# GitHubOfAndrew/TeAMOFlow

Hardware: AMD Instinct MI355X
Metric: train_interactions_per_sec (higher is better)
Workload: dtype f32

## Files before the change

teamoflow_amd/csrc/tmf_wmrb.hip:

```cpp
#include <math.h>
#include <stdlib.h>

#include <type_traits>

#include "tmf_common.h"

namespace tmf {

constexpr int kThreads = 256;
constexpr int kWaves = kThreads / 64;
constexpr int kPosChunk = 512;
constexpr int kUnrollW = 4;
constexpr int kG4Unroll = 4;

__host__ __device__ inline int round4(int x) { return (x + 3) & ~3; }

__host__ __device__ inline int sp_padded(int S) {
    const int nf4 = (S + 3) / 4;
    const int per = ((nf4 + 2 * kWaves - 1) / (2 * kWaves) + 1) & ~1;
    return 4 * 2 * kWaves * per;
}

__device__ __forceinline__ void count_ge0_x4(int& c0, int& c1, float x0, float x1, float x2, float x3) {
    unsigned long long m0, m1, m2, m3;
// ... 995 lines not shown
__global__ __launch_bounds__(64 * (kS5Waves + 1)) void k_wmrb_scores5(const int32_t* __restrict__ ids, const int32_t* __restrict__ outs,
                                                                     const int64_t* __restrict__ wg_ptr, int64_t wg0, int64_t n_users,
                                                                     const T* __restrict__ U, const T* __restrict__ V,
                                                                     float* __restrict__ sp, float* __restrict__ p, S5Pace pace) {
    constexpr int G = 32, NGB = 2 * kS5Waves;
    constexpr uint32_t RB = RowBytes<G, NV, T>::value;
    extern __shared__ __attribute__((aligned(16))) char smem_raw[];
    __shared__ int s_win[kS5Waves];
    __shared__ int s_gate;
    int* wst = reinterpret_cast<int*>(smem_raw + (size_t)kS5Users * RB);
    const int tid = threadIdx.x, lane = tid & 63, wave = tid >> 6, g = lane & (G - 1), gid = tid / G;
    const int64_t wg = wg0 + blockIdx.x;
    const int64_t ubeg = wg * kS5Users;
    const int nu = (int)((n_users - ubeg < kS5Users) ? n_users - ubeg : kS5Users);
    const bool paced = pace.cnt != nullptr;
    {
        const tmf_f4* src = reinterpret_cast<const tmf_f4*>(reinterpret_cast<const char*>(U) + ubeg * (int64_t)RB);
        tmf_f4* dst = reinterpret_cast<tmf_f4*>(smem_raw);
        for (int i = tid; i < nu * (int)(RB / 16); i += 64 * (kS5Waves + 1)) dst[i] = __builtin_nontemporal_load(src + i);
        if (paced)
            for (int i = tid; i <= pace.nw; i += 64 * (kS5Waves + 1)) wst[i] = pace.wst[wg * (pace.nw + 1) + i];
        if (tid < kS5Waves) s_win[tid] = 0;
        if (tid == 0) s_gate = paced ? pace.lag : INT32_MAX;
    }
    __syncthreads();
    if (wave == kS5Waves) {
        if (!paced) return;
        const int x = blockIdx.x & 7, peers = ((int)gridDim.x - x + 7) / 8;
        int* cnt = pace.cnt + (size_t)x * pace.nw * kS5Stride;
        int published = 0, gate = pace.lag, idle = 0;
        bool open = false;
        for (;;) {
            int mn = (lane < kS5Waves) ? __hip_atomic_load(&s_win[lane], __ATOMIC_RELAXED, __HIP_MEMORY_SCOPE_WORKGROUP) : INT32_MAX;
#pragma unroll
            for (int o = 8; o >= 1; o >>= 1) mn = min(mn, __shfl_xor(mn, o, 64));
            mn = __builtin_amdgcn_readfirstlane(mn);
            const bool done = mn == INT32_MAX;
            const int target = done ? pace.nw : mn;
            if (lane == 0)
                for (int w = published; w < target; ++w) __hip_atomic_fetch_add(cnt + (size_t)w * kS5Stride, 1, __ATOMIC_RELAXED, __HIP_MEMORY_SCOPE_AGENT);
            if (target > published) published = target;
            if (done) return;
            if (!open && gate < pace.nw - 1) {
                int c = (lane == 0) ? __hip_atomic_load(cnt + (size_t)(gate - pace.lag) * kS5Stride, __ATOMIC_RELAXED, __HIP_MEMORY_SCOPE_AGENT) : 0;
                c = __builtin_amdgcn_readfirstlane(c);
                if (c >= peers) {
                    ++gate;
                    idle = 0;
                    if (lane == 0) __hip_atomic_store(&s_gate, gate, __ATOMIC_RELAXED, __HIP_MEMORY_SCOPE_WORKGROUP);
                    continue;
                }
                if (++idle > 4000) {
                    open = true;
                    if (lane == 0) __hip_atomic_store(&s_gate, INT32_MAX, __ATOMIC_RELAXED, __HIP_MEMORY_SCOPE_WORKGROUP);
                }
            }
            __builtin_amdgcn_s_sleep(4);
        }
    }
    const int64_t beg = wg_ptr[wg], end = wg_ptr[wg + 1];
    const int steps = (int)((end - beg) >> 3);
    const uint32_t loff = 16u * (uint32_t)g;
    const int my_entry = Reduce8x32::entry_of_lane(lane);
    const bool owner = Reduce8x32::owner(lane);
    const int4* id4 = reinterpret_cast<const int4*>(ids + beg);
    const int32_t* out8 = outs + beg + my_entry;
    const int mine = steps > gid ? (steps - gid + NGB - 1) / NGB : 0;
    const int rounds = __builtin_amdgcn_readfirstlane(mine);
    if (rounds > 0) {
        const int last = mine > 0 ? gid + NGB * (mine - 1) : 0;
        struct Ids {
            int4 a, b;
            int o;
        };
        auto fetch = [&](int i) {
            const int st = gid + NGB * i;
            const int sc = st <= last ? st : last;
            Ids r{id4[2 * sc], id4[2 * sc + 1], out8[8 * sc]};
            if (i >= mine) r.o = kS5Pad;
            return r;
        };
        int cur_w = 0, next_b = paced ? wst[1] : INT32_MAX;
        auto pace_to = [&](int i) {
            if (!paced || i >= rounds || cur_w >= pace.nw - 1) return;
            const int st_w = __builtin_amdgcn_readfirstlane(gid + NGB * i);
            if (st_w < next_b) return;
            do {
                ++cur_w;
                next_b = wst[cur_w + 1];
            } while (st_w >= next_b && cur_w < pace.nw - 1);
            if (lane == 0) __hip_atomic_store(&s_win[wave], cur_w, __ATOMIC_RELAXED, __HIP_MEMORY_SCOPE_WORKGROUP);
            for (int spin = 0; spin < 20000; ++spin) {
                if (__hip_atomic_load(&s_gate, __ATOMIC_RELAXED, __HIP_MEMORY_SCOPE_WORKGROUP) >= cur_w) break;
                __builtin_amdgcn_s_sleep(2);
            }
        };
        auto gather = [&](Raw<NV, T> (&y)[8], const Ids& d) {
            const int idv[8] = {d.a.x, d.a.y, d.a.z, d.a.w, d.b.x, d.b.y, d.b.z, d.b.w};
#pragma unroll
            for (int t = 0; t < 8; ++t) load_raw32<G, NV>(y[t], V, (uint32_t)idv[t] & 0xffffffu, loff);
        };
        auto finish = [&](const Raw<NV, T> (&y)[8], const Ids& d) {
            const int idv[8] = {d.a.x, d.a.y, d.a.z, d.a.w, d.b.x, d.b.y, d.b.z, d.b.w};
            float pr[8];
#pragma unroll
            for (int t = 0; t < 8; ++t) {
                Raw<NV, T> x;
                const char* xr = smem_raw + ((uint32_t)idv[t] >> 24) * RB + loff;
                if constexpr (std::is_same<T, float>::value) {
#pragma unroll
                    for (int v = 0; v < NV; ++v) x.v[v] = *reinterpret_cast<const float4*>(xr + 16 * G * v);
                } else {
#pragma unroll
                    for (int pv = 0; pv < NV / 2; ++pv) x.v[pv] = *reinterpret_cast<const bf16x8*>(xr + 16 * G * pv);
                }
                pr[t] = dot_raw<NV>(x, y[t]);
            }
            const float sc = Reduce8x32::run(pr, lane);
            if (owner && d.o != kS5Pad) __builtin_nontemporal_store(sc, d.o >= 0 ? sp + d.o : p + ~d.o);
        };
        Raw<NV, T> yA[8], yB[8];
        Ids A = fetch(0);
        Ids B = fetch(1);
        pace_to(0);
        gather(yA, A);
        for (int i = 0; i < rounds; i += 2) {
            Ids C = fetch(i + 2);
            __builtin_amdgcn_sched_barrier(0);
            pace_to(i + 1);
            gather(yB, B);
            __builtin_amdgcn_sched_barrier(0);
            finish(yA, A);
            __builtin_amdgcn_sched_barrier(0);
            if (i + 1 >= rounds) break;
            Ids Dn = fetch(i + 3);
            __builtin_amdgcn_sched_barrier(0);
            pace_to(i + 2);
            gather(yA, C);
            __builtin_amdgcn_sched_barrier(0);
            finish(yB, B);
            __builtin_amdgcn_sched_barrier(0);
            A = C;
            B = Dn;
        }
    }
    if (lane == 0) __hip_atomic_store(&s_win[wave], INT32_MAX, __ATOMIC_RELAXED, __HIP_MEMORY_SCOPE_WORKGROUP);
}

}

namespace tmf {
constexpr int kS6Users = 64;
constexpr int kS6Waves = 8;

template <int NV, typename T>
__global__ __launch_bounds__(64 * kS6Waves) void k_wmrb_scores6(const int32_t* __restrict__ ids, const int32_t* __restrict__ outs,
                                                                const int64_t* __restrict__ chunk_ptr, int64_t chunk0, int64_t n_groups,
                                                                int64_t n_users, const T* __restrict__ U, const T* __restrict__ V,
                                                                float* __restrict__ sp, float* __restrict__ p) {
    constexpr int G = 32, NGB = 2 * kS6Waves;
    constexpr uint32_t RB = RowBytes<G, NV, T>::value;
    __shared__ __attribute__((aligned(16))) char smem_raw[kS6Users * RB];
    const int tid = threadIdx.x, lane = tid & 63, g = lane & (G - 1), gid = tid / G;
    const int64_t chunk = chunk0 + blockIdx.x;
    const int64_t beg = chunk_ptr[chunk], end = chunk_ptr[chunk + 1];
    if (beg == end) return;
    const int64_t ubeg = (chunk % n_groups) * kS6Users;
    const int nu = (int)((n_users - ubeg < kS6Users) ? n_users - ubeg : kS6Users);
    {
        const tmf_f4* src = reinterpret_cast<const tmf_f4*>(reinterpret_cast<const char*>(U) + ubeg * (int64_t)RB);
        tmf_f4* dst = reinterpret_cast<tmf_f4*>(smem_raw);
        for (int i = tid; i < nu * (int)(RB / 16); i += 64 * kS6Waves) dst[i] = __builtin_nontemporal_load(src + i);
    }
    __syncthreads();
    const int steps = (int)((end - beg) >> 3);
    const uint32_t loff = 16u * (uint32_t)g;
    const int my_entry = Reduce8x32::entry_of_lane(lane);
    const bool owner = Reduce8x32::owner(lane);
    const int4* id4 = reinterpret_cast<const int4*>(ids + beg);
    const int32_t* out8 = outs + beg + my_entry;
    const int mine = steps > gid ? (steps - gid + NGB - 1) / NGB : 0;
    const int rounds = __builtin_amdgcn_readfirstlane(mine);
    if (rounds == 0) return;
    const int last = mine > 0 ? gid + NGB * (mine - 1) : 0;
    struct Ids {
        int4 a, b;
        int o;
    };
    auto fetch = [&](int i) {
        const int st = gid + NGB * i;
        const int sc = st <= last ? st : last;
        Ids r{id4[2 * sc], id4[2 * sc + 1], out8[8 * sc]};
        if (i >= mine) r.o = kS5Pad;
        return r;
    };
    auto gather = [&](Raw<NV, T> (&y)[8], const Ids& d) {
        const int idv[8] = {d.a.x, d.a.y, d.a.z, d.a.w, d.b.x, d.b.y, d.b.z, d.b.w};
#pragma unroll
        for (int t = 0; t < 8; ++t) load_raw32<G, NV>(y[t], V, (uint32_t)idv[t] & 0xffffffu, loff);
    };
    auto finish = [&](const Raw<NV, T> (&y)[8], const Ids& d) {
        const int idv[8] = {d.a.x, d.a.y, d.a.z, d.a.w, d.b.x, d.b.y, d.b.z, d.b.w};
        float pr[8];
#pragma unroll
        for (int t = 0; t < 8; ++t) {
            Raw<NV, T> x;
            const char* xr = smem_raw + ((uint32_t)idv[t] >> 24) * RB + loff;
            if constexpr (std::is_same<T, float>::value) {
#pragma unroll
                for (int v = 0; v < NV; ++v) x.v[v] = *reinterpret_cast<const float4*>(xr + 16 * G * v);
            } else {
#pragma unroll
                for (int pv = 0; pv < NV / 2; ++pv) x.v[pv] = *reinterpret_cast<const bf16x8*>(xr + 16 * G * pv);
            }
            pr[t] = dot_raw<NV>(x, y[t]);
        }
        const float sc = Reduce8x32::run(pr, lane);
        if (owner && d.o != kS5Pad) __builtin_nontemporal_store(sc, d.o >= 0 ? sp + d.o : p + ~d.o);
    };
    Raw<NV, T> yA[8];
    Ids A = fetch(0);
    for (int i = 0; i < rounds; ++i) {
        Ids B = fetch(i + 1);
        __builtin_amdgcn_sched_barrier(0);
        gather(yA, A);
        __builtin_amdgcn_sched_barrier(0);
        finish(yA, A);
        A = B;
    }
}

}

static bool s6_supported(int n_components, int bf16, int64_t n_items) {
    const tmf::RowGeom geom = bf16 ? tmf::row_geom_bf16(n_components) : tmf::row_geom(n_components);
    const int64_t row_bytes = (int64_t)geom.ld * (bf16 ? 2 : 4);
    return geom.G == 32 && n_items > 0 && n_items < (1 << 24) && n_items * row_bytes < ((int64_t)1 << 32);
}

template <typename T>
static int wmrb_scores6_impl(const int32_t* ids, const int32_t* outs, const int64_t* chunk_ptr, int64_t n_groups, int32_t n_slices,
                             int64_t n_users, int64_t n_items, const void* U, const void* V, float* sp, float* p, int n_components,
                             void* stream) {
    if (n_users == 0 || n_slices == 0) return TMF_OK;
    const RowGeom geom = row_geom_of<T>(n_components);
    TMF_REQUIRE(ids && outs && chunk_ptr && U && V && sp && p, "wmrb_scores6: null pointer");
    TMF_REQUIRE(n_groups == (n_users + kS6Users - 1) / kS6Users && n_slices > 0, "wmrb_scores6: %lld groups for %lld users (%d per group), %d slices",
                (long long)n_groups, (long long)n_users, kS6Users, n_slices);
    if (!s6_supported(n_components, std::is_same<T, __bf16>::value, n_items)) {
        set_error("wmrb_scores6: needs rows of 32 lanes (fp32 65..128 / bf16 129..256 components) and fewer than 2^24 items in a table "
                  "below 4 GB (got %d components, %lld items)", n_components, (long long)n_items);
        return TMF_E_UNSUPPORTED;
    }
    const int64_t per_slice = n_groups * 64 * kS6Waves;
    const int max_slices = (int)((((int64_t)1 << 32) - 1) / per_slice);
    TMF_REQUIRE(max_slices >= 1, "wmrb_scores6: %lld user groups exceed one launch", (long long)n_groups);
    for (int s0 = 0; s0 < n_slices; s0 += max_slices) {
        const int nsl = (n_slices - s0 < max_slices) ? n_slices - s0 : max_slices;
        const unsigned blocks = (unsigned)(n_groups * nsl);
#define CALL(G_, NV_)                                                                                                       \
    {                                                                                                                       \
        if constexpr (G_ == 32) {                                                                                           \
            hipLaunchKernelGGL((k_wmrb_scores6<NV_, T>), dim3(blocks), dim3(64 * kS6Waves), 0, (hipStream_t)stream, ids, outs, \
                               chunk_ptr, (int64_t)s0 * n_groups, n_groups, n_users, (const T*)U, (const T*)V, sp, p);      \
        }                                                                                                                   \
    }
        TMF_DISPATCH(T, geom, CALL);
#undef CALL
    }
    return check_launch("tmf_wmrb_scores6");
}

namespace tmf {
constexpr int kS7Users = 256;
constexpr int kS7Slots = 6144;
constexpr int kS7K = 4;
constexpr int kS7Waves = 16;
constexpr int kS7Flight = 2;
constexpr uint32_t kS7RowBytes = 512;
constexpr size_t kS7Lds = (size_t)kS7Users * kS7RowBytes + (size_t)(kS7Slots + 64) * sizeof(float);

struct S7Streams {
    const int4* steps;
    const int32_t* place;
    const int64_t* sub_step;
    const int64_t* sub_place;
    const int32_t* chunk_sub;
    const int32_t* sub_wave;
    const int32_t* sub_fill;
};

__global__ __launch_bounds__(64 * kS7Waves) void k_wmrb_scores7(S7Streams a, int64_t chunk0, int64_t n_groups, int64_t n_users,
                                                                const float* __restrict__ U, const float* __restrict__ V,
                                                                float* __restrict__ sp, float* __restrict__ p) {
    constexpr int NG = 8 * kS7Waves, NT = 64 * kS7Waves, FL = kS7Flight;
    extern __shared__ __attribute__((aligned(16))) char smem_raw[];
    float* sbuf = reinterpret_cast<float*>(smem_raw + (size_t)kS7Users * kS7RowBytes);
    const int tid = threadIdx.x, lane = tid & 63, g = lane & 7, gid = tid >> 3;
    const int64_t chunk = chunk0 + blockIdx.x;
    const int sub_b = a.chunk_sub[chunk], sub_e = a.chunk_sub[chunk + 1];
    if (sub_b == sub_e) return;
    const int64_t ubeg = (chunk % n_groups) * kS7Users;
    const int nu = (int)((n_users - ubeg < kS7Users) ? n_users - ubeg : kS7Users);
    {
        const tmf_f4* src = reinterpret_cast<const tmf_f4*>(reinterpret_cast<const char*>(U) + ubeg * (int64_t)kS7RowBytes);
        tmf_f4* dst = reinterpret_cast<tmf_f4*>(smem_raw);
        for (int i = tid; i < nu * (int)(kS7RowBytes / 16); i += NT) dst[i] = __builtin_nontemporal_load(src + i);
    }
    __syncthreads();
    const uint32_t par = (lane >> 4) & 1;
    const uint32_t offA = 16u * g + 128u * par, offB = 16u * g + 128u * (par ^ 1u);
    const uint32_t slot_sel = 0x0c0c0000u | ((2u * (g & 3) + 1u) << 8) | (2u * (g & 3));
    struct Row {
        float4 v[4];
    };
    auto dot = [](const Row& x, const Row& y) {
        float q[4];
#pragma unroll
        for (int v = 0; v < 4; ++v) {
            tmf_f2 a = tmf_f2{x.v[v].x, x.v[v].y} * tmf_f2{y.v[v].x, y.v[v].y};
            a = __builtin_elementwise_fma(tmf_f2{x.v[v].z, x.v[v].w}, tmf_f2{y.v[v].z, y.v[v].w}, a);
            q[v] = a.x + a.y;
        }
        return (q[0] + q[2]) + (q[1] + q[3]);
    };
    auto run = [&](auto fill_tag, const int4* rec0, int first, int stride, int end, int rounds) {
        constexpr int FILL = decltype(fill_tag)::value;
        auto fetch = [&](int i) {
            const int st = first + stride * i;
            return rec0[st < end ? st : end - 1];
        };
        auto gather = [&](Row& y, const int4& r) {
            const char* base = reinterpret_cast<const char*>(V);
            const uint32_t oa = row_byte_off<kS7RowBytes>((uint32_t)r.x, offA), ob = row_byte_off<kS7RowBytes>((uint32_t)r.x, offB);
            y.v[0] = *reinterpret_cast<const float4*>(base + oa);
            y.v[1] = *reinterpret_cast<const float4*>(base + ob);
            y.v[2] = *reinterpret_cast<const float4*>(base + oa + 256);
            y.v[3] = *reinterpret_cast<const float4*>(base + ob + 256);
        };
        auto finish = [&](const Row& y, const int4& r, int i) {
            float s[FILL];
#pragma unroll
            for (int k = 0; k < FILL; ++k) {
                const uint32_t lu = ((uint32_t)r.y >> (8 * k)) & 0xffu;
                const char* xa = smem_raw + (lu * kS7RowBytes + offA);
                const char* xb = smem_raw + (lu * kS7RowBytes + offB);
                Row x;
                x.v[0] = *reinterpret_cast<const float4*>(xa);
                x.v[1] = *reinterpret_cast<const float4*>(xb);
                x.v[2] = *reinterpret_cast<const float4*>(xa + 256);
                x.v[3] = *reinterpret_cast<const float4*>(xb + 256);
                float t = dot(x, y);
                t += TMF_DPP_MOV(t, 0xB1);
                t += TMF_DPP_MOV(t, 0x4E);
                t += TMF_DPP_MOV(t, 0x141);
                s[k] = t;
            }
            float mine_s = s[0];
            if constexpr (FILL == 2) mine_s = (g & 1) ? s[1] : s[0];
            if constexpr (FILL == 3) mine_s = (g & 2) ? s[2] : ((g & 1) ? s[1] : s[0]);
            if constexpr (FILL == 4) mine_s = (g & 2) ? ((g & 1) ? s[3] : s[2]) : ((g & 1) ? s[1] : s[0]);
            uint32_t slot = __builtin_amdgcn_perm((uint32_t)r.w, (uint32_t)r.z, slot_sel);
            slot = (slot < (uint32_t)kS7Slots && first + stride * i < end) ? slot : (uint32_t)kS7Slots;
            if (g < FILL) sbuf[slot] = mine_s;
        };
        Row y[FL];
        int4 rec[2 * FL];
#pragma unroll
        for (int j = 0; j < FL; ++j) rec[j] = fetch(j);
#pragma unroll
        for (int j = 0; j < FL; ++j) {
            gather(y[j], rec[j]);
            rec[FL + j] = fetch(FL + j);
        }
        int i = 0;
        for (; i + 2 * FL <= rounds; i += 2 * FL) {
#pragma unroll
            for (int j = 0; j < 2 * FL; ++j) {
                __builtin_amdgcn_sched_barrier(0);
                finish(y[j % FL], rec[j], i + j);
                __builtin_amdgcn_sched_barrier(0);
                gather(y[j % FL], rec[(j + FL) % (2 * FL)]);
                rec[j] = fetch(i + j + 2 * FL);
            }
        }
        const int rem = rounds - i;
#pragma unroll
        for (int j = 0; j < 2 * FL - 1; ++j) {
            if (j < rem) {
                __builtin_amdgcn_sched_barrier(0);
                finish(y[j % FL], rec[j], i + j);
                __builtin_amdgcn_sched_barrier(0);
                if (j + FL < rem) gather(y[j % FL], rec[j + FL]);
            }
        }
    };
    const int wave = __builtin_amdgcn_readfirstlane(tid >> 6);
    const bool by_fill = a.sub_wave != nullptr;
    for (int sub = sub_b; sub < sub_e; ++sub) {
        const int64_t st0 = a.sub_step[sub];
        const int nsteps = (int)(a.sub_step[sub + 1] - st0);
        const int64_t pl0 = a.sub_place[sub];
        const int nslots = (int)(a.sub_place[sub + 1] - pl0);
        const int4* rec0 = a.steps + st0;
        const int32_t* pl = a.place + pl0;
        int32_t where[kS7Slots / NT];
#pragma unroll
        for (int q = 0; q < kS7Slots / NT; ++q) where[q] = (tid + NT * q < nslots) ? __builtin_nontemporal_load(pl + tid + NT * q) : 0;
        int lo = 8 * wave, hi = nsteps, stride = NG, wb = 0, we = 0, cls = 0;
        if (by_fill) {
            const int32_t* sw = a.sub_wave + (int64_t)sub * (kS7Waves + 1) + wave;
            wb = __builtin_amdgcn_readfirstlane(sw[0]);
            we = __builtin_amdgcn_readfirstlane(sw[1]);
            cls = __builtin_amdgcn_readfirstlane(a.sub_fill[(int64_t)sub * kS7K]);
            lo = wb, hi = we < cls ? we : cls, stride = 8;
        }
        if (lo < hi) run(std::integral_constant<int, 4>{}, rec0, lo + (by_fill ? (gid & 7) : gid - 8 * wave), stride, hi, (hi - lo + stride - 1) / stride);
        if (by_fill) {
            const int32_t* sf = a.sub_fill + (int64_t)sub * kS7K;
            int end = cls + __builtin_amdgcn_readfirstlane(sf[1]);
            lo = wb > cls ? wb : cls, hi = we < end ? we : end, cls = end;
            if (lo < hi) run(std::integral_constant<int, 3>{}, rec0, lo + (gid & 7), 8, hi, (hi - lo + 7) / 8);
            end = cls + __builtin_amdgcn_readfirstlane(sf[2]);
            lo = wb > cls ? wb : cls, hi = we < end ? we : end, cls = end;
            if (lo < hi) run(std::integral_constant<int, 2>{}, rec0, lo + (gid & 7), 8, hi, (hi - lo + 7) / 8);
            lo = wb > cls ? wb : cls, hi = we;
            if (lo < hi) run(std::integral_constant<int, 1>{}, rec0, lo + (gid & 7), 8, hi, (hi - lo + 7) / 8);
        }
        __syncthreads();
#pragma unroll
        for (int q = 0; q < kS7Slots / NT; ++q)
            if (tid + NT * q < nslots)
                __builtin_nontemporal_store(sbuf[tid + NT * q], where[q] >= 0 ? sp + where[q] : p + ~where[q]);
        __syncthreads();
    }
}

}

static bool s7_supported(int n_components, int bf16, int64_t n_items) {
    return !bf16 && n_components >= 65 && n_components <= 128 && s6_supported(n_components, 0, n_items);
}

static int wmrb_scores7_impl(const void* steps, const int32_t* place, const int64_t* sub_step, const int64_t* sub_place,
                             const int32_t* chunk_sub, const int32_t* sub_wave, const int32_t* sub_fill, int64_t n_groups, int32_t n_slices, int64_t n_users, int64_t n_items,
                             const void* U, const void* V, float* sp, float* p, int n_components, void* stream) {
    if (n_users == 0 || n_slices == 0) return TMF_OK;
    TMF_REQUIRE(steps && place && sub_step && sub_place && chunk_sub && U && V && sp && p, "wmrb_scores7: null pointer");
    TMF_REQUIRE(!sub_wave == !sub_fill, "wmrb_scores7: sub_wave and sub_fill come together");
    TMF_REQUIRE(n_groups == (n_users + kS7Users - 1) / kS7Users && n_slices > 0, "wmrb_scores7: %lld groups for %lld users (%d per group), %d slices",
                (long long)n_groups, (long long)n_users, kS7Users, n_slices);
    if (!s7_supported(n_components, 0, n_items)) {
        set_error("wmrb_scores7: needs fp32 rows of 65..128 components and fewer than 2^24 items in a table below 4 GB "
                  "(got %d components, %lld items)", n_components, (long long)n_items);
        return TMF_E_UNSUPPORTED;
    }
    static LdsGrant grant;
    if (int rc = grant_dynamic_lds(reinterpret_cast<const void*>(&k_wmrb_scores7), kS7Lds, grant)) return rc;
    const S7Streams a{static_cast<const int4*>(steps), place, sub_step, sub_place, chunk_sub, sub_wave, sub_fill};
    const int64_t per_slice = n_groups * 64 * kS7Waves;
    const int max_slices = (int)((((int64_t)1 << 32) - 1) / per_slice);
    TMF_REQUIRE(max_slices >= 1, "wmrb_scores7: %lld user groups exceed one launch", (long long)n_groups);
    for (int s0 = 0; s0 < n_slices; s0 += max_slices) {
        const int nsl = (n_slices - s0 < max_slices) ? n_slices - s0 : max_slices;
        hipLaunchKernelGGL(k_wmrb_scores7, dim3((unsigned)(n_groups * nsl)), dim3(64 * kS7Waves), kS7Lds, (hipStream_t)stream, a,
                           (int64_t)s0 * n_groups, n_groups, n_users, (const float*)U, (const float*)V, sp, p);
    }
    return check_launch("tmf_wmrb_scores7");
}

static int s5_launches(int64_t n_wg, int wgs_per_launch) { return (int)((n_wg + wgs_per_launch - 1) / wgs_per_launch); }
static int s5_wgs_per_launch(int wgs_per_launch) {
    if (wgs_per_launch > 0) return wgs_per_launch;
    int dev = 0, cus = 256;
    if (hipGetDevice(&dev) == hipSuccess) (void)hipDeviceGetAttribute(&cus, hipDeviceAttributeMultiprocessorCount, dev);
    return cus > 0 ? cus : 256;
}

template <typename T>
static int wmrb_scores5_impl(const int32_t* ids, const int32_t* outs, const int64_t* wg_ptr, int64_t n_wg, int64_t n_users,
                             int64_t n_items, const void* U, const void* V, float* sp, float* p, int n_components,
                             int wgs_per_launch, const int32_t* wstart, int32_t n_windows, int lag, void* workspace,
                             size_t workspace_bytes, void* stream) {
    if (n_wg == 0 || n_users == 0) return TMF_OK;
    const RowGeom geom = row_geom_of<T>(n_components);
    TMF_REQUIRE(ids && outs && wg_ptr && U && V && sp && p, "wmrb_scores5: null pointer");
    TMF_REQUIRE(n_wg == (n_users + kS5Users - 1) / kS5Users, "wmrb_scores5: %lld workgroups for %lld users (%d per workgroup)",
                (long long)n_wg, (long long)n_users, kS5Users);
    const size_t row_bytes = (size_t)geom.ld * sizeof(T);
    if (geom.G != 32 || row_bytes * kS5Users > 128 * 1024 || n_items <= 0 || n_items >= (1 << 24) ||
        (int64_t)n_items * (int64_t)row_bytes >= ((int64_t)1 << 32)) {
        set_error("wmrb_scores5: needs rows of 32 lanes (fp32 65..128 / bf16 129..256 components) and fewer than 2^24 items "
                  "in a table below 4 GB (got %d components, %lld items)", n_components, (long long)n_items);
        return TMF_E_UNSUPPORTED;
    }
    wgs_per_launch = s5_wgs_per_launch(wgs_per_launch);
    const int launches = s5_launches(n_wg, wgs_per_launch);
    const bool paced = wstart != nullptr && workspace != nullptr && n_windows > 1;
    const size_t per_launch = (size_t)8 * (paced ? n_windows : 0) * kS5Stride * sizeof(int);
    if (paced) {
        TMF_REQUIRE(n_windows <= kS5MaxWindows && lag >= 0, "wmrb_scores5: %d windows (at most %d), lag %d", n_windows, kS5MaxWindows, lag);
        TMF_REQUIRE(workspace_bytes >= per_launch * launches, "wmrb_scores5: workspace of %zu bytes needed, got %zu", per_launch * launches,
                    workspace_bytes);
        if (hipMemsetAsync(workspace, 0, per_launch * launches, (hipStream_t)stream) != hipSuccess) {
            set_error("wmrb_scores5: hipMemsetAsync failed");
            return TMF_E_LAUNCH;
        }
    }
    const size_t lds = row_bytes * kS5Users + (paced ? (size_t)(n_windows + 1) * sizeof(int) : 0);
#define CALL(G_, NV_)                                                                                                       \
    {                                                                                                                       \
        if constexpr (G_ == 32) {                                                                                           \
            static LdsGrant grant;                                                                                          \
            if (int rc = grant_dynamic_lds(reinterpret_cast<const void*>(&k_wmrb_scores5<NV_, T>), lds, grant)) return rc;  \
            for (int l = 0; l < launches; ++l) {                                                                            \
                const int64_t w0 = (int64_t)l * wgs_per_launch;                                                             \
                const unsigned blocks = (unsigned)((n_wg - w0 < wgs_per_launch) ? n_wg - w0 : wgs_per_launch);              \
                const S5Pace pace{wstart, paced ? reinterpret_cast<int*>(static_cast<char*>(workspace) + per_launch * l) : nullptr, \
                                  n_windows, lag};                                                                          \
                hipLaunchKernelGGL((k_wmrb_scores5<NV_, T>), dim3(blocks), dim3(64 * (kS5Waves + 1)), lds, (hipStream_t)stream, \
                                   ids, outs, wg_ptr, w0, n_users, (const T*)U, (const T*)V, sp, p, pace);                  \
            }                                                                                                               \
        }                                                                                                                   \
    }
    TMF_DISPATCH(T, geom, CALL);
#undef CALL
    return check_launch("tmf_wmrb_scores5");
}

template <typename T>
static int wmrb_finish_impl(const float* part, int32_t n_slices, int32_t n_users, const void* U_old, void* U_out,
                            int n_components, int epi, tmf_adam adam, void* stream) {
    if (n_users == 0) return TMF_OK;
    TMF_REQUIRE(part && U_out && n_slices > 0 && (epi == TMF_EPI_GRAD || U_old), "wmrb_finish: bad arguments");
    TMF_REQUIRE(epi == TMF_EPI_ADAM || epi == TMF_EPI_GRAD, "wmrb_finish: bad epilogue %d", epi);
    const RowGeom geom = row_geom_of<T>(n_components);
#define CALL(G_, NV_)                                                                                                  \
    {                                                                                                                  \
        constexpr int per_block = (64 / G_) * kWaves;                                                                  \
        hipLaunchKernelGGL((k_wmrb_finish<G_, NV_, T>), dim3((unsigned)(((int64_t)n_users + per_block - 1) / per_block)), \
                           dim3(kThreads), 0, (hipStream_t)stream, part, (int)n_slices, (int64_t)n_users,                \
                           (const T*)U_old, U_out, epi, adam);                                                         \
    }
    TMF_DISPATCH(T, geom, CALL);
#undef CALL
    return check_launch("tmf_wmrb_finish");
}

#define TMF_SLICED_ENTRY_POINTS(SFX, T_)                                                                                  \
    extern "C" int tmf_wmrb_scores3_##SFX(const tmf_slice_lists* lists, const void* U, const void* V, float* sp, float* p, \
                                          int n_components, void* stream) {                                               \
        return wmrb_scores3_impl<T_>(lists, U, V, sp, p, n_components, stream);                                           \
    }                                                                                                                     \
    extern "C" int tmf_wmrb_scores5_##SFX(const int32_t* ids, const int32_t* outs, const int64_t* wg_ptr, int64_t n_wg,    \
                                          int64_t n_users, int64_t n_items, const void* U, const void* V, float* sp,      \
                                          float* p, int n_components, int wgs_per_launch, const int32_t* wstart,          \
                                          int32_t n_windows, int lag, void* workspace, size_t workspace_bytes,            \
                                          void* stream) {                                                                 \
        return wmrb_scores5_impl<T_>(ids, outs, wg_ptr, n_wg, n_users, n_items, U, V, sp, p, n_components, wgs_per_launch, \
                                     wstart, n_windows, lag, workspace, workspace_bytes, stream);                         \
    }                                                                                                                     \
    extern "C" int tmf_wmrb_scores6_##SFX(const int32_t* ids, const int32_t* outs, const int64_t* chunk_ptr, int64_t n_groups, \
                                          int32_t n_slices, int64_t n_users, int64_t n_items, const void* U, const void* V, \
                                          float* sp, float* p, int n_components, void* stream) {                          \
        return wmrb_scores6_impl<T_>(ids, outs, chunk_ptr, n_groups, n_slices, n_users, n_items, U, V, sp, p, n_components, stream); \
    }                                                                                                                     \
    extern "C" int tmf_wmrb_gradu3_##SFX(const tmf_slice_lists* lists, const float* D, const float* delta,                \
                                         const void* V, float* part, int per_slice_launches, int n_components,            \
                                         void* stream) {                                                                  \
        return wmrb_gradu3_impl<T_>(lists, D, delta, V, part, per_slice_launches, n_components, stream);                  \
    }                                                                                                                     \
    extern "C" int tmf_wmrb_gradu4_##SFX(const tmf_slice_lists* lists, const float* D, const float* delta, const void* V,  \
                                         const void* U_old, void* U_out, int n_components, int epi, tmf_adam adam,       \
                                         int32_t users_per_launch, void* workspace, size_t workspace_bytes, void* stream) { \
        return wmrb_gradu4_impl<T_>(lists, D, delta, V, U_old, U_out, n_components, epi, adam, users_per_launch, workspace, \
                                    workspace_bytes, stream);                                                            \
    }                                                                                                                     \
    extern "C" int tmf_wmrb_finish_##SFX(const float* part, int32_t n_slices, int32_t n_users, const void* U_old,         \
                                         void* U_out, int n_components, int epi, tmf_adam adam, void* stream) {           \
        return wmrb_finish_impl<T_>(part, n_slices, n_users, U_old, U_out, n_components, epi, adam, stream);               \
    }

TMF_SLICED_ENTRY_POINTS(f32, float)
TMF_SLICED_ENTRY_POINTS(bf16, __bf16)

extern "C" int tmf_wmrb_scores6_users_per_group(void) { return tmf::kS6Users; }
extern "C" int tmf_wmrb_scores6_supported(int n_components, int bf16, int64_t n_items) { return s6_supported(n_components, bf16, n_items); }
extern "C" int tmf_wmrb_scores7_f32(const void* steps, const int32_t* place, const int64_t* sub_step, const int64_t* sub_place,
                                    const int32_t* chunk_sub, int64_t n_groups, int32_t n_slices, int64_t n_users, int64_t n_items,
                                    const void* U, const void* V, float* sp, float* p, int n_components, void* stream) {
    return wmrb_scores7_impl(steps, place, sub_step, sub_place, chunk_sub, nullptr, nullptr, n_groups, n_slices, n_users, n_items, U, V, sp, p,
                             n_components, stream);
}
extern "C" int tmf_wmrb_scores7_fill_f32(const void* steps, const int32_t* place, const int64_t* sub_step, const int64_t* sub_place,
                                         const int32_t* chunk_sub, const int32_t* sub_wave, const int32_t* sub_fill, int64_t n_groups,
                                         int32_t n_slices, int64_t n_users, int64_t n_items, const void* U, const void* V, float* sp,
                                         float* p, int n_components, void* stream) {
    TMF_REQUIRE(sub_wave && sub_fill, "wmrb_scores7_fill: null pointer");
    return wmrb_scores7_impl(steps, place, sub_step, sub_place, chunk_sub, sub_wave, sub_fill, n_groups, n_slices, n_users, n_items, U, V,
                             sp, p, n_components, stream);
}
extern "C" int tmf_wmrb_scores7_waves(void) { return tmf::kS7Waves; }
extern "C" int tmf_wmrb_scores7_users_per_group(void) { return tmf::kS7Users; }
extern "C" int tmf_wmrb_scores7_slots(void) { return tmf::kS7Slots; }
extern "C" int tmf_wmrb_scores7_supported(int n_components, int bf16, int64_t n_items) { return s7_supported(n_components, bf16, n_items); }
extern "C" int tmf_wmrb_scores5_users_per_workgroup(void) { return tmf::kS5Users; }
extern "C" size_t tmf_wmrb_scores5_workspace_bytes(int64_t n_wg, int32_t n_windows, int wgs_per_launch) {
    if (n_wg <= 0 || n_windows <= 1) return 0;
    return (size_t)s5_launches(n_wg, s5_wgs_per_launch(wgs_per_launch)) * 8 * (size_t)n_windows * tmf::kS5Stride * sizeof(int);
}
extern "C" int tmf_wmrb_scores5_supported(int n_components, int bf16, int64_t n_items) {
    const tmf::RowGeom geom = bf16 ? tmf::row_geom_bf16(n_components) : tmf::row_geom(n_components);
    const int64_t row_bytes = (int64_t)geom.ld * (bf16 ? 2 : 4);
    return geom.G == 32 && row_bytes * tmf::kS5Users <= 128 * 1024 && n_items > 0 && n_items < (1 << 24) &&
           n_items * row_bytes < ((int64_t)1 << 32);
}
```

Before: 1.302 billion.

## Software-pipeline sub-batches and overlap user staging with record and row prefetch

```diff
diff --git a/teamoflow_amd/csrc/tmf_wmrb.hip b/teamoflow_amd/csrc/tmf_wmrb.hip
--- a/teamoflow_amd/csrc/tmf_wmrb.hip
+++ b/teamoflow_amd/csrc/tmf_wmrb.hip
@@ -1321,15 +1321,9 @@
     if (sub_b == sub_e) return;
     const int64_t ubeg = (chunk % n_groups) * kS7Users;
     const int nu = (int)((n_users - ubeg < kS7Users) ? n_users - ubeg : kS7Users);
-    {
-        const tmf_f4* src = reinterpret_cast<const tmf_f4*>(reinterpret_cast<const char*>(U) + ubeg * (int64_t)kS7RowBytes);
-        tmf_f4* dst = reinterpret_cast<tmf_f4*>(smem_raw);
-        for (int i = tid; i < nu * (int)(kS7RowBytes / 16); i += NT) dst[i] = __builtin_nontemporal_load(src + i);
-    }
-    __syncthreads();
     const uint32_t par = (lane >> 4) & 1;
     const uint32_t offA = 16u * g + 128u * par, offB = 16u * g + 128u * (par ^ 1u);
-    const uint32_t slot_sel = 0x0c0c0000u | ((2u * (g & 3) + 1u) << 8) | (2u * (g & 3));
+    const uint32_t slot_sel = 0x0c0c0000u | ((2u * (g & 1) + 1u) << 8) | (2u * (g & 1));
     struct Row {
         float4 v[4];
     };
@@ -1343,115 +1337,182 @@
         }
         return (q[0] + q[2]) + (q[1] + q[3]);
     };
-    auto run = [&](auto fill_tag, const int4* rec0, int first, int stride, int end, int rounds) {
+    const int wave = __builtin_amdgcn_readfirstlane(tid >> 6);
+    const bool by_fill = a.sub_wave != nullptr;
+    const int stride = by_fill ? 8 : NG;
+    struct Sub {
+        const int4* rec0;
+        const int32_t* pl;
+        int nslots;
+        int first, end;
+        int rounds;
+        int r4, r3, r2;
+    };
+    auto scalars = [&](int sub) {
+        Sub s;
+        const int32_t* none = reinterpret_cast<const int32_t*>(a.sub_step + sub);
+        const int32_t* sw = by_fill ? a.sub_wave + (int64_t)sub * (kS7Waves + 1) + wave : none;
+        const int32_t* sf = by_fill ? a.sub_fill + (int64_t)sub * kS7K : none;
+        const int64_t st0 = a.sub_step[sub], st1 = a.sub_step[sub + 1], pl0 = a.sub_place[sub], pl1 = a.sub_place[sub + 1];
+        const int wb = __builtin_amdgcn_readfirstlane(sw[0]), we = __builtin_amdgcn_readfirstlane(sw[1]);
+        const int f4 = __builtin_amdgcn_readfirstlane(sf[0]), f3 = __builtin_amdgcn_readfirstlane(sf[1]);
+        const int f2 = __builtin_amdgcn_readfirstlane(sf[2]);
+        const int nsteps = (int)(st1 - st0);
+        s.rec0 = a.steps + st0;
+        s.pl = a.place + pl0;
+        s.nslots = (int)(pl1 - pl0);
+        const int lo = by_fill ? wb : 8 * wave, hi = by_fill ? we : nsteps, shift = by_fill ? 3 : 7;
+        static_assert(NG == 1 << 7, "rounds of the round-robin form");
+        const int c4 = by_fill ? f4 : nsteps, c3 = by_fill ? c4 + f3 : nsteps, c2 = by_fill ? c3 + f2 : nsteps;
+        auto upto = [&](int c) {
+            const int h = hi < c ? hi : c;
+            return h > lo ? (h - lo + stride - 1) >> shift : 0;
+        };
+        s.first = by_fill ? wb + (gid & 7) : gid, s.end = hi, s.rounds = upto(hi);
+        s.r4 = upto(c4), s.r3 = upto(c3), s.r2 = upto(c2);
+        return s;
+    };
+    auto fetch = [&](const Sub& s, int i) {
+        const int st = s.first + stride * i, last = s.end > 0 ? s.end - 1 : 0;
+        return reinterpret_cast<const int32_t*>(s.rec0 + (st < s.end ? st : last))[g & 3];
+    };
+    auto word = [](int32_t w, auto ctrl) { return (uint32_t)__builtin_amdgcn_update_dpp(0, w, decltype(ctrl)::value, 0xf, 0xf, false); };
+    constexpr std::integral_constant<int, 0x00> kX{};
+    constexpr std::integral_constant<int, 0x55> kY{};
+    constexpr std::integral_constant<int, 0xFA> kZW{};
+    auto gather = [&](Row& y, int32_t r) {
+        const char* base = reinterpret_cast<const char*>(V);
+        const uint32_t item = word(r, kX);
+        const uint32_t oa = row_byte_off<kS7RowBytes>(item, offA), ob = row_byte_off<kS7RowBytes>(item, offB);
+        y.v[0] = *reinterpret_cast<const float4*>(base + oa);
+        y.v[1] = *reinterpret_cast<const float4*>(base + ob);
+        y.v[2] = *reinterpret_cast<const float4*>(base + oa + 256);
+        y.v[3] = *reinterpret_cast<const float4*>(base + ob + 256);
+    };
+    auto finish = [&](auto fill_tag, const Sub& sc, const Row& y, int32_t r, int i) {
         constexpr int FILL = decltype(fill_tag)::value;
-        auto fetch = [&](int i) {
-            const int st = first + stride * i;
-            return rec0[st < end ? st : end - 1];
-        };
-        auto gather = [&](Row& y, const int4& r) {
-            const char* base = reinterpret_cast<const char*>(V);
-            const uint32_t oa = row_byte_off<kS7RowBytes>((uint32_t)r.x, offA), ob = row_byte_off<kS7RowBytes>((uint32_t)r.x, offB);
-            y.v[0] = *reinterpret_cast<const float4*>(base + oa);
-            y.v[1] = *reinterpret_cast<const float4*>(base + ob);
-            y.v[2] = *reinterpret_cast<const float4*>(base + oa + 256);
-            y.v[3] = *reinterpret_cast<const float4*>(base + ob + 256);
-        };
-        auto finish = [&](const Row& y, const int4& r, int i) {
-            float s[FILL];
-#pragma unroll
-            for (int k = 0; k < FILL; ++k) {
-                const uint32_t lu = ((uint32_t)r.y >> (8 * k)) & 0xffu;
-                const char* xa = smem_raw + (lu * kS7RowBytes + offA);
-                const char* xb = smem_raw + (lu * kS7RowBytes + offB);
-                Row x;
-                x.v[0] = *reinterpret_cast<const float4*>(xa);
-                x.v[1] = *reinterpret_cast<const float4*>(xb);
-                x.v[2] = *reinterpret_cast<const float4*>(xa + 256);
-                x.v[3] = *reinterpret_cast<const float4*>(xb + 256);
-                float t = dot(x, y);
-                t += TMF_DPP_MOV(t, 0xB1);
-                t += TMF_DPP_MOV(t, 0x4E);
-                t += TMF_DPP_MOV(t, 0x141);
-                s[k] = t;
-            }
-            float mine_s = s[0];
-            if constexpr (FILL == 2) mine_s = (g & 1) ? s[1] : s[0];
-            if constexpr (FILL == 3) mine_s = (g & 2) ? s[2] : ((g & 1) ? s[1] : s[0]);
-            if constexpr (FILL == 4) mine_s = (g & 2) ? ((g & 1) ? s[3] : s[2]) : ((g & 1) ? s[1] : s[0]);
-            uint32_t slot = __builtin_amdgcn_perm((uint32_t)r.w, (uint32_t)r.z, slot_sel);
-            slot = (slot < (uint32_t)kS7Slots && first + stride * i < end) ? slot : (uint32_t)kS7Slots;
-            if (g < FILL) sbuf[slot] = mine_s;
-        };
-        Row y[FL];
-        int4 rec[2 * FL];
-#pragma unroll
-        for (int j = 0; j < FL; ++j) rec[j] = fetch(j);
-#pragma unroll
-        for (int j = 0; j < FL; ++j) {
-            gather(y[j], rec[j]);
-            rec[FL + j] = fetch(FL + j);
-        }
-        int i = 0;
-        for (; i + 2 * FL <= rounds; i += 2 * FL) {
+        const uint32_t users = word(r, kY);
+        float s[FILL];
+#pragma unroll
+        for (int k = 0; k < FILL; ++k) {
+            const uint32_t lu = (users >> (8 * k)) & 0xffu;
+            const char* xa = smem_raw + (lu * kS7RowBytes + offA);
+            const char* xb = smem_raw + (lu * kS7RowBytes + offB);
+            Row x;
+            x.v[0] = *reinterpret_cast<const float4*>(xa);
+            x.v[1] = *reinterpret_cast<const float4*>(xb);
+            x.v[2] = *reinterpret_cast<const float4*>(xa + 256);
+            x.v[3] = *reinterpret_cast<const float4*>(xb + 256);
+            float t = dot(x, y);
+            t += TMF_DPP_MOV(t, 0xB1);
+            t += TMF_DPP_MOV(t, 0x4E);
+            t += TMF_DPP_MOV(t, 0x141);
+            s[k] = t;
+        }
+        float mine_s = s[0];
+        if constexpr (FILL == 2) mine_s = (g & 1) ? s[1] : s[0];
+        if constexpr (FILL == 3) mine_s = (g & 2) ? s[2] : ((g & 1) ? s[1] : s[0]);
+        if constexpr (FILL == 4) mine_s = (g & 2) ? ((g & 1) ? s[3] : s[2]) : ((g & 1) ? s[1] : s[0]);
+        uint32_t slot = __builtin_amdgcn_perm(0u, word(r, kZW), slot_sel);
+        slot = (slot < (uint32_t)kS7Slots && sc.first + stride * i < sc.end) ? slot : (uint32_t)kS7Slots;
+        if (g < FILL) sbuf[slot] = mine_s;
+    };
+    Row y[FL];
+    int32_t rec[2 * FL];
+    constexpr int NQ = kS7Slots / NT;
+    auto ask_places = [&](int32_t(&w)[NQ], const Sub& s) {
+#pragma unroll
+        for (int q = 0; q < NQ; ++q) {
+            const int idx = tid + NT * q;
+            w[q] = __builtin_nontemporal_load(s.pl + (idx < s.nslots ? idx : s.nslots - 1));
+        }
+    };
+    auto ask_records = [&](const Sub& s) {
+#pragma unroll
+        for (int j = 0; j < 2 * FL; ++j) rec[j] = fetch(s, j);
+    };
+    auto ask_rows = [&]() {
+#pragma unroll
+        for (int j = 0; j < FL; ++j) gather(y[j], rec[j]);
+    };
+    auto rings = [&](auto fill_tag, const Sub& s, int& i, int upto) {
+        for (; i < upto; i += 2 * FL) {
 #pragma unroll
             for (int j = 0; j < 2 * FL; ++j) {
                 __builtin_amdgcn_sched_barrier(0);
-                finish(y[j % FL], rec[j], i + j);
+                finish(fill_tag, s, y[j % FL], rec[j], i + j);
                 __builtin_amdgcn_sched_barrier(0);
                 gather(y[j % FL], rec[(j + FL) % (2 * FL)]);
-                rec[j] = fetch(i + j + 2 * FL);
-            }
-        }
-        const int rem = rounds - i;
+                rec[j] = fetch(s, i + j + 2 * FL);
+            }
+        }
+    };
+    auto tail = [&](auto fill_tag, const Sub& s, int i) {
+        const int rem = s.rounds - i;
 #pragma unroll
         for (int j = 0; j < 2 * FL - 1; ++j) {
             if (j < rem) {
                 __builtin_amdgcn_sched_barrier(0);
-                finish(y[j % FL], rec[j], i + j);
+                finish(fill_tag, s, y[j % FL], rec[j], i + j);
                 __builtin_amdgcn_sched_barrier(0);
                 if (j + FL < rem) gather(y[j % FL], rec[j + FL]);
             }
         }
     };
-    const int wave = __builtin_amdgcn_readfirstlane(tid >> 6);
-    const bool by_fill = a.sub_wave != nullptr;
+    Sub cur = scalars(sub_b);
+    {
+        constexpr int NP = kS7Users * (int)(kS7RowBytes / 16) / NT;
+        const tmf_f4* src = reinterpret_cast<const tmf_f4*>(reinterpret_cast<const char*>(U) + ubeg * (int64_t)kS7RowBytes);
+        tmf_f4* dst = reinterpret_cast<tmf_f4*>(smem_raw);
+        const int lim = nu * (int)(kS7RowBytes / 16);
+        tmf_f4 piece[NP];
+#pragma unroll
+        for (int q = 0; q < NP; ++q) piece[q] = __builtin_nontemporal_load(src + (tid + NT * q < lim ? tid + NT * q : lim - 1));
+        ask_records(cur);
+#pragma unroll
+        for (int q = 0; q < NP; ++q) dst[tid + NT * q] = piece[q];
+        ask_rows();
+    }
+    __syncthreads();
     for (int sub = sub_b; sub < sub_e; ++sub) {
-        const int64_t st0 = a.sub_step[sub];
-        const int nsteps = (int)(a.sub_step[sub + 1] - st0);
-        const int64_t pl0 = a.sub_place[sub];
-        const int nslots = (int)(a.sub_place[sub + 1] - pl0);
-        const int4* rec0 = a.steps + st0;
-        const int32_t* pl = a.place + pl0;
-        int32_t where[kS7Slots / NT];
-#pragma unroll
-        for (int q = 0; q < kS7Slots / NT; ++q) where[q] = (tid + NT * q < nslots) ? __builtin_nontemporal_load(pl + tid + NT * q) : 0;
-        int lo = 8 * wave, hi = nsteps, stride = NG, wb = 0, we = 0, cls = 0;
-        if (by_fill) {
-            const int32_t* sw = a.sub_wave + (int64_t)sub * (kS7Waves + 1) + wave;
-            wb = __builtin_amdgcn_readfirstlane(sw[0]);
-            we = __builtin_amdgcn_readfirstlane(sw[1]);
-            cls = __builtin_amdgcn_readfirstlane(a.sub_fill[(int64_t)sub * kS7K]);
-            lo = wb, hi = we < cls ? we : cls, stride = 8;
-        }
-        if (lo < hi) run(std::integral_constant<int, 4>{}, rec0, lo + (by_fill ? (gid & 7) : gid - 8 * wave), stride, hi, (hi - lo + stride - 1) / stride);
-        if (by_fill) {
-            const int32_t* sf = a.sub_fill + (int64_t)sub * kS7K;
-            int end = cls + __builtin_amdgcn_readfirstlane(sf[1]);
-            lo = wb > cls ? wb : cls, hi = we < end ? we : end, cls = end;
-            if (lo < hi) run(std::integral_constant<int, 3>{}, rec0, lo + (gid & 7), 8, hi, (hi - lo + 7) / 8);
-            end = cls + __builtin_amdgcn_readfirstlane(sf[2]);
-            lo = wb > cls ? wb : cls, hi = we < end ? we : end, cls = end;
-            if (lo < hi) run(std::integral_constant<int, 2>{}, rec0, lo + (gid & 7), 8, hi, (hi - lo + 7) / 8);
-            lo = wb > cls ? wb : cls, hi = we;
-            if (lo < hi) run(std::integral_constant<int, 1>{}, rec0, lo + (gid & 7), 8, hi, (hi - lo + 7) / 8);
-        }
+        const Sub nxt = scalars(sub + 1 < sub_e ? sub + 1 : sub);
+        constexpr int RING = 2 * FL;
+        const int full = cur.rounds & ~(RING - 1);
+        auto ring_end = [&](int r) {
+            const int e = (r + RING - 1) & ~(RING - 1);
+            return e < full ? e : full;
+        };
+        int i = 0;
+        rings(std::integral_constant<int, 4>{}, cur, i, ring_end(cur.r4));
+        rings(std::integral_constant<int, 3>{}, cur, i, ring_end(cur.r3));
+        rings(std::integral_constant<int, 2>{}, cur, i, ring_end(cur.r2));
+        rings(std::integral_constant<int, 1>{}, cur, i, full);
+        if (full < cur.rounds) {
+            if (full < cur.r4) tail(std::integral_constant<int, 4>{}, cur, full);
+            else if (full < cur.r3) tail(std::integral_constant<int, 3>{}, cur, full);
+            else if (full < cur.r2) tail(std::integral_constant<int, 2>{}, cur, full);
+            else tail(std::integral_constant<int, 1>{}, cur, full);
+        }
+        int32_t where[NQ];
+        ask_places(where, cur);
+        ask_records(nxt);
+        __builtin_amdgcn_sched_barrier(0);
         __syncthreads();
-#pragma unroll
-        for (int q = 0; q < kS7Slots / NT; ++q)
-            if (tid + NT * q < nslots)
-                __builtin_nontemporal_store(sbuf[tid + NT * q], where[q] >= 0 ? sp + where[q] : p + ~where[q]);
+        __builtin_amdgcn_sched_barrier(0);
+        float val[NQ];
+        float* to[NQ];
+#pragma unroll
+        for (int q = 0; q < NQ; ++q) {
+            const int idx = tid + NT * q;
+            val[q] = sbuf[idx < cur.nslots ? idx : cur.nslots - 1];
+            to[q] = where[q] >= 0 ? sp + where[q] : p + ~where[q];
+        }
+        ask_rows();
+#pragma unroll
+        for (int q = 0; q < NQ; ++q)
+            if (tid + NT * q < cur.nslots) __builtin_nontemporal_store(val[q], to[q]);
         __syncthreads();
+        cur = nxt;
     }
 }
 
```

Result: no change. 1.315 billion, median of 6 (+1.0%).
